# ValentinoGuerrini/Configurable-Hierarchical-Allreduce-Algorithms

Measured on AMD Instinct MI355X. Metric: device-resident bucket-reduction GB/s (fp32); allreduce GB/s at 2/4/8 GPUs, higher is better.
Workload: dtype f32; 1 GPU; C2 bucket reduction: k=2 (m=1 incoming bucket), 64 MiB fp32 per bucket, device-resident, MPI_Reduce_local semantics; bucket_bytes=67108864, m=1, buffer_sets=16, parallelism=replicas, gate=untimed spin kernel ahead of the start event

## Files before the change

### configurable-hierarchical-allreduce-algorithms_amd/csrc/reduce_kernels.hip

```cpp
#include <hip/hip_runtime.h>

#include <algorithm>

#include <cstdlib>

#include "reduce_vec.hpp"

namespace chr {

int& coresident_depth() {
    static thread_local int depth = 0;
    return depth;
}

ReduceTuning& reduce_tuning() {
    static ReduceTuning t = [] {
        ReduceTuning r;
        const char* s = std::getenv("CHR_REDUCE_MAX_LAUNCH_VEC");
        r.max_launch_vec = s ? (size_t)std::atoll(s) : 0;
        s = std::getenv("CHR_XCD_RUN_KIB");
        r.xcd_run_kib = s ? std::atoi(s) : -1;
        s = std::getenv("CHR_REDUCE_NT");
        r.nt_mode = s ? std::atoi(s) : -1;
        s = std::getenv("CHR_REDUCE_NT_MIN_BYTES");
        r.nt_min_bytes = s ? (size_t)std::atoll(s) : (size_t)40 << 20;
        r.tree_nt_min_bytes = s ? r.nt_min_bytes : (size_t)64 << 20;
        s = std::getenv("CHR_WG_PER_CU_VEC");
        r.wg_per_cu_vec = s ? std::max(0, std::atoi(s)) : -1;
        s = std::getenv("CHR_WG_PER_CU_TREE");
        r.wg_per_cu_tree = s ? std::max(0, std::atoi(s)) : -1;
        s = std::getenv("CHR_XCD_HAND_SHIFT");
        r.xcd_hand_shift = s ? std::min(31, std::max(0, std::atoi(s))) : -1;
        int dev = 0, lds = 0, blk = 0;
        if (hipGetDevice(&dev) != hipSuccess ||
            hipDeviceGetAttribute(&lds, hipDeviceAttributeMaxSharedMemoryPerMultiprocessor, dev) != hipSuccess ||
            lds <= 0)
            lds = 0;
        if (hipDeviceGetAttribute(&blk, hipDeviceAttributeMaxSharedMemoryPerBlock, dev) != hipSuccess || blk <= 0)
            blk = 0;
        r.lds_per_cu = (unsigned)lds;
        r.lds_per_block = (unsigned)blk;
        return r;
    }();
    return t;
}


static hipError_t launch_vec(const VecArgs& a, int kdt, int kop, int m, hipStream_t s) {
    kdt = vec_kernel_dt(kdt, kop);
    switch (kernel_tu(false, kdt, kop)) {
    case kTuCore: return launch_vec_tu<kTuCore>(a, kdt, kop, m, s);
    case kTuInt: return launch_vec_int(a, kdt, kop, m, s);
    case kTuPair: return launch_vec_pair(a, kdt, kop, m, s);
    default: return hipErrorInvalidValue;
    }
}

static hipError_t launch_scalar(void* out, const void* acc, const void* const* ins, int m, size_t n, int kdt,
                                int kop, hipStream_t s) {
    if (n == 0) return hipSuccess;
    ScalarArgs a{};
    a.out = out;
    a.acc = acc;
    a.m = m;
    a.n = n;
    for (int j = 0; j < m; ++j) a.ins[j] = ins[j];
    switch (kernel_tu(false, kdt, kop)) {
    case kTuCore: return launch_scalar_tu<kTuCore>(a, kdt, kop, s);
    case kTuInt: return launch_scalar_int(a, kdt, kop, s);
    case kTuPair: return launch_scalar_pair(a, kdt, kop, s);
    default: return hipErrorInvalidValue;
    }
}

static hipError_t launch_group(void* out, const void* acc, const void* const* ins, int m, size_t n, int dtype,
                               int op, hipStream_t s) {
    const size_t es = dtype_size(dtype);
    const void* operands[kMaxFanIn + 1] = {acc};
    for (int j = 0; j < m; ++j) operands[j + 1] = ins[j];
    const AlignSplit sp = align_split(out, operands, m + 1, n, es);
    if (!sp.congruent) return launch_scalar(out, acc, ins, m, n, dtype, op, s);
    hipError_t err;
    if (sp.head && (err = launch_scalar(out, acc, ins, m, sp.head, dtype, op, s)) != hipSuccess) return err;
    if (sp.nvec) {
        VecArgs a{};
        a.out = (u32x4*)((char*)out + sp.head * es);
        a.acc = (const u32x4*)((const char*)acc + sp.head * es);
        for (int j = 0; j < m; ++j) a.ins[j] = (const u32x4*)((const char*)ins[j] + sp.head * es);
        a.nvec = sp.nvec;
        if ((err = launch_vec(a, dtype, op, m, s)) != hipSuccess) return err;
    }
    if (sp.tail) {
        const size_t o = (n - sp.tail) * es;
        const void* tins[kMaxFanIn];
        for (int j = 0; j < m; ++j) tins[j] = (const char*)ins[j] + o;
        return launch_scalar((char*)out + o, (const char*)acc + o, tins, m, sp.tail, dtype, op, s);
    }
    return hipSuccess;
}

hipError_t launch_reduce(void* out, const void* acc, const void* const* ins, int m, size_t n, int dtype, int op,
                         hipStream_t stream, bool running_first) {
    if (n == 0) return hipSuccess;
    if (!valid_dtype_op(dtype, op)) return hipErrorInvalidValue;
    const size_t es = dtype_size(dtype);
    const KernelId k = canon_op(dtype, op, running_first);
    dtype = k.dt, op = k.op;
    if (m == 0) {
        if (out == acc) return hipSuccess;
        return hipMemcpyAsync(out, acc, n * es, hipMemcpyDeviceToDevice, stream);
    }
    for (int j0 = 0; j0 < m; j0 += kMaxFanIn) {
        const int mg = (m - j0) < kMaxFanIn ? (m - j0) : kMaxFanIn;
        hipError_t err = launch_group(out, j0 == 0 ? acc : out, ins + j0, mg, n, dtype, op, stream);
        if (err != hipSuccess) return err;
    }
    return hipSuccess;
}


__device__ __forceinline__ uint64_t splitmix64(uint64_t x) {
    x += 0x9E3779B97F4A7C15ull;
    x = (x ^ (x >> 30)) * 0xBF58476D1CE4E5B9ull;
    x = (x ^ (x >> 27)) * 0x94D049BB133111EBull;
    return x ^ (x >> 31);
}

__device__ __forceinline__ float gen_f32(uint64_t seed, uint64_t rank, uint64_t i) {
    return (float)(splitmix64(seed ^ (rank << 40) ^ i) >> 40) * (1.0f / 8388608.0f) - 1.0f;
}
__device__ __forceinline__ double gen_f64(uint64_t seed, uint64_t rank, uint64_t i) {
    return (double)(splitmix64(seed ^ (rank << 40) ^ i) >> 11) * (1.0 / 4503599627370496.0) - 1.0;
}

__device__ void fill_pair(char* elem, int dtype, int pattern, uint64_t seed, uint64_t rank, uint64_t count_for_seq,
                          uint64_t g) {
    const float ft[8] = {0.0f, -0.0f, 1.0f, -1.0f, 0.0f, -0.0f, 0.5f, 0.0f};
    const uint64_t key = splitmix64(seed ^ (rank << 40) ^ g);
    const unsigned sel = (unsigned)(key >> 61);
    const uint32_t pay = (uint32_t)(rank + 1) & 0x3Fu;
    const int32_t small = (int32_t)(key >> 61) - 4;
    const int32_t idx = pattern == 1 ? (int32_t)rank : (int32_t)((key >> 32) & 0x3F);
    const int32_t seq = (int32_t)(uint32_t)(rank * count_for_seq + g);
    uint32_t w[4] = {0, 0, 0, 0};
    switch (dtype) {
    case CHR_FLOAT_INT: {
        const float v = pattern == 1 ? (float)seq : pattern == 2 ? ft[sel] : (float)small;
        w[0] = pattern == 2 && sel == 7 ? (0x7FC00000u | (pay << 16) | pay) : __float_as_uint(v);
        w[1] = (uint32_t)idx;
        break;
    }
    case CHR_DOUBLE_INT: {
        const double v = pattern == 1 ? (double)seq : pattern == 2 ? (double)ft[sel] : (double)small;
        const uint64_t u = pattern == 2 && sel == 7 ? (0x7FF8000000000000ull | ((uint64_t)pay << 40) | pay)
                                                     : (uint64_t)__double_as_longlong(v);
        w[0] = (uint32_t)u;
        w[1] = (uint32_t)(u >> 32);
        w[2] = (uint32_t)idx;
        break;
    }
    case CHR_LONG_INT: {
        const uint64_t u = (uint64_t)(int64_t)(pattern == 1 ? seq : small);
        w[0] = (uint32_t)u;
        w[1] = (uint32_t)(u >> 32);
        w[2] = (uint32_t)idx;
        break;
    }
    case CHR_2INT:
        w[0] = (uint32_t)(pattern == 1 ? seq : small);
        w[1] = (uint32_t)idx;
        break;
    case CHR_SHORT_INT:
        w[0] = (uint32_t)(uint16_t)(int16_t)(pattern == 1 ? seq : small);
        w[1] = (uint32_t)idx;
        break;
    case CHR_C_FLOAT_COMPLEX: {
        const float re = pattern == 1 ? (float)seq : pattern == 2 ? ft[sel] : gen_f32(seed, rank, 2 * g);
        const float im = pattern == 1 ? -(float)seq : pattern == 2 ? ft[(key >> 58) & 7] : gen_f32(seed, rank, 2 * g + 1);
        w[0] = __float_as_uint(re);
        w[1] = __float_as_uint(im);
        break;
    }
    default: {
        const double re = pattern == 1 ? (double)seq : pattern == 2 ? (double)ft[sel] : gen_f64(seed, rank, 2 * g);
        const double im = pattern == 1 ? -(double)seq : pattern == 2 ? (double)ft[(key >> 58) & 7]
                                                                     : gen_f64(seed, rank, 2 * g + 1);
        const uint64_t ur = (uint64_t)__double_as_longlong(re), ui = (uint64_t)__double_as_longlong(im);
        w[0] = (uint32_t)ur;
        w[1] = (uint32_t)(ur >> 32);
        w[2] = (uint32_t)ui;
        w[3] = (uint32_t)(ui >> 32);
        break;
    }
    }
    const int nw = dtype == CHR_DOUBLE_INT || dtype == CHR_LONG_INT || dtype == CHR_C_DOUBLE_COMPLEX ? 4 : 2;
    for (int k = 0; k < nw; ++k) ((uint32_t*)elem)[k] = w[k];
}

__global__ __launch_bounds__(kBlock) void k_fill(void* buf, size_t n, int dtype, int pattern, uint64_t seed,
                                                 uint64_t rank, uint64_t count_for_seq) {
    if (dtype >= CHR_FLOAT_INT) {
        const size_t es = dtype == CHR_DOUBLE_INT || dtype == CHR_LONG_INT || dtype == CHR_C_DOUBLE_COMPLEX ? 16 : 8;
        for (size_t i = (size_t)blockIdx.x * kBlock + threadIdx.x; i < n; i += (size_t)gridDim.x * kBlock)
            fill_pair((char*)buf + i * es, dtype, pattern, seed, rank, count_for_seq, i);
        return;
    }
    const int es = dtype == CHR_INT8 || dtype == CHR_UINT8 ? 1 : dtype == CHR_INT16 || dtype == CHR_UINT16 ? 2
                   : dtype == CHR_UINT32 || (dtype == CHR_INT32 && pattern == 3) ? 4
                   : dtype == CHR_INT64 || dtype == CHR_UINT64 ? 8 : 0;
    for (size_t i = (size_t)blockIdx.x * kBlock + threadIdx.x; i < n; i += (size_t)gridDim.x * kBlock) {
        if (es) {
            const uint64_t u = splitmix64(seed ^ (rank << 40) ^ (uint64_t)i);
            const unsigned sel = (unsigned)(u >> 61);
            const uint64_t v = pattern == 1   ? rank * count_for_seq + i
                               : pattern == 2 ? (uint64_t)(int64_t)(sel == 6 ? 2 : sel == 7 ? 7 : sel == 2 ? 1
                                                                    : sel == 3 ? -1 : 0)
                               : pattern == 3 ? (sel ? (u >> (64 - 8 * es)) | 1u : 0)
                                              : u >> (64 - 8 * es);
            if (es == 1) ((uint8_t*)buf)[i] = (uint8_t)v;
            else if (es == 2) ((uint16_t*)buf)[i] = (uint16_t)v;
            else if (es == 4) ((uint32_t*)buf)[i] = (uint32_t)v;
            else ((uint64_t*)buf)[i] = v;
            continue;
        }
        if (pattern == 1) {
            const int32_t v = (int32_t)(uint32_t)(rank * count_for_seq + i);
            switch (dtype) {
            case CHR_FLOAT32: ((float*)buf)[i] = (float)v; break;
            case CHR_FLOAT64: ((double*)buf)[i] = (double)v; break;
            case CHR_INT32: ((int32_t*)buf)[i] = v; break;
            default: ((uint16_t*)buf)[i] = f2bf((float)v); break;
            }
        } else if (pattern == 2) {
            const unsigned sel = (unsigned)(splitmix64(seed ^ (rank << 40) ^ (uint64_t)i) >> 61);
            const uint32_t pay = (uint32_t)(rank + 1) & 0x3Fu;
            const float fv = sel == 2 ? 1.0f : sel == 3 ? -1.0f : sel == 6 ? 0.5f : (sel & 1) ? -0.0f : 0.0f;
            switch (dtype) {
            case CHR_FLOAT32:
                ((uint32_t*)buf)[i] = sel == 7 ? (0x7FC00000u | (pay << 16) | pay) : __float_as_uint(fv);
                break;
            case CHR_FLOAT64:
                ((uint64_t*)buf)[i] = sel == 7 ? (0x7FF8000000000000ull | ((uint64_t)pay << 40) | pay)
                                               : (uint64_t)__double_as_longlong((double)fv);
                break;
            case CHR_INT32: ((int32_t*)buf)[i] = sel == 6 ? 2 : sel == 7 ? 7 : sel == 2 ? 1 : sel == 3 ? -1 : 0; break;
            default: ((uint16_t*)buf)[i] = sel == 7 ? (uint16_t)(0x7FC0u | pay) : f2bf(fv); break;
            }
        } else {
            const uint64_t u = splitmix64(seed ^ (rank << 40) ^ (uint64_t)i);
            switch (dtype) {
            case CHR_FLOAT32: ((float*)buf)[i] = (float)(u >> 40) * (1.0f / 8388608.0f) - 1.0f; break;
            case CHR_FLOAT64: ((double*)buf)[i] = (double)(u >> 11) * (1.0 / 4503599627370496.0) - 1.0; break;
            case CHR_INT32: ((int32_t*)buf)[i] = (int32_t)(uint32_t)(u >> 32); break;
            default: ((uint16_t*)buf)[i] = f2bf((float)(u >> 40) * (1.0f / 8388608.0f) - 1.0f); break;
            }
        }
    }
}

hipError_t launch_fill(void* buf, size_t n, int dtype, int pattern, uint64_t seed, int rank, uint64_t count_for_seq,
                       hipStream_t stream) {
    if (n == 0) return hipSuccess;
    const size_t trips = (n + kBlock - 1) / kBlock;
    const int grid = (int)(trips < 8192 ? trips : 8192);
    hipLaunchKernelGGL(k_fill, dim3(grid), dim3(kBlock), 0, stream, buf, n, dtype, pattern, seed, (uint64_t)rank,
                       count_for_seq);
    return hipGetLastError();
}

}
```

### configurable-hierarchical-allreduce-algorithms_amd/csrc/reduce_tree.hip

```cpp
#include <hip/hip_runtime.h>

#include "reduce_tree.hpp"

namespace chr {

static hipError_t launch_tree_any(const TreeArgs& a, const TreeScalarArgs* sa, int kdt, int kop, hipStream_t s) {
    if (!sa) kdt = vec_kernel_dt(kdt, kop);
    switch (kernel_tu(true, kdt, kop)) {
    case kTuTree: return launch_tree_tu<kTuTree>(a, sa, kdt, kop, s);
    case kTuTreeIntNarrow: return launch_tree_int_narrow(a, sa, kdt, kop, s);
    case kTuTreeIntWide: return launch_tree_int_wide(a, sa, kdt, kop, s);
    case kTuTreePair: return launch_tree_pair(a, sa, kdt, kop, s);
    default: return hipErrorInvalidValue;
    }
}

bool tree_program_ok(int nl, const uint8_t* comb, const uint8_t* swaps, uint32_t* comb_bits, uint32_t* swap_bits) {
    if (nl < 1 || nl > kMaxLeaves || !comb) return false;
    int d = 0, nc = 0;
    uint32_t cb = 0, sb = 0;
    for (int j = 0; j < nl; ++j) {
        if (++d > kTreeDepth) return false;
        if ((int)comb[j] > d - 1) return false;
        cb |= (uint32_t)comb[j] << (2 * j);
        for (int c = 0; c < comb[j]; ++c, ++nc) {
            if (swaps && swaps[nc]) sb |= 1u << nc;
            --d;
        }
    }
    if (d != 1 || nc != nl - 1) return false;
    *comb_bits = cb;
    *swap_bits = sb;
    return true;
}

hipError_t launch_reduce_tree_multi(const TreeJob* jobs, int njobs, int dtype, int op, hipStream_t stream) {
    if (!valid_dtype_op(dtype, op)) return hipErrorInvalidValue;
    const size_t es = dtype_size(dtype);
    const int dtype0 = dtype, op0 = op;
    const KernelId k = canon_op(dtype, op, false);
    dtype = k.dt, op = k.op;
    TreeArgs pend[kMaxLeaves + 1] = {};
    auto flush = [&](int nl) -> hipError_t {
        TreeArgs& a = pend[nl];
        if (!a.nseg) return hipSuccess;
        a.nl = nl;
        const hipError_t e = launch_tree_any(a, nullptr, dtype, op, stream);
        a.nseg = 0;
        return e;
    };
    for (int t = 0; t < njobs; ++t) {
        const TreeJob& jb = jobs[t];
        if (jb.n == 0) continue;
        uint32_t cb = 0, sb = 0;
        if (!tree_program_ok(jb.nl, jb.comb, jb.swaps, &cb, &sb)) return hipErrorInvalidValue;
        const int nl = jb.nl;
        if (nl == 1) {
            if (jb.out != jb.leaves[0]) {
                const hipError_t e = hipMemcpyAsync(jb.out, jb.leaves[0], jb.n * es, hipMemcpyDeviceToDevice, stream);
                if (e != hipSuccess) return e;
            }
            continue;
        }
        if (nl == 2 && 3 * jb.n * es >= reduce_tuning().nt_min_bytes) {
            const bool sw = (sb & 1u) != 0;
            const void* acc = jb.leaves[sw ? 1 : 0];
            const void* in = jb.leaves[sw ? 0 : 1];
            if (jb.out != in) {
                const hipError_t e = launch_reduce(jb.out, acc, &in, 1, jb.n, dtype0, op0, stream);
                if (e != hipSuccess) return e;
                continue;
            }
        }
        const AlignSplit sp = align_split(jb.out, jb.leaves, nl, jb.n, es);
        const size_t head = sp.head, nvec = sp.nvec;
        auto scalar = [&](size_t off, size_t cnt) -> hipError_t {
            if (!cnt) return hipSuccess;
            TreeScalarArgs sa{};
            sa.out = (char*)jb.out + off * es;
            for (int j = 0; j < nl; ++j) sa.leaves[j] = (const char*)jb.leaves[j] + off * es;
            sa.n = cnt;
            sa.nl = nl;
            sa.comb = cb;
            sa.swaps = sb;
            TreeArgs dummy{};
            return launch_tree_any(dummy, &sa, dtype, op, stream);
        };
        hipError_t err;
        if (!sp.congruent) {
            if ((err = scalar(0, jb.n)) != hipSuccess) return err;
            continue;
        }
        if ((err = scalar(0, head)) != hipSuccess || (err = scalar(jb.n - sp.tail, sp.tail)) != hipSuccess) return err;
        const size_t cap = reduce_tuning().max_launch_vec;
        const size_t seg_cap = cap && cap < kMaxSegVec ? cap : kMaxSegVec;
        for (size_t off = 0; off < nvec; off += seg_cap) {
            TreeArgs& a = pend[nl];
            TreeSeg& g = a.seg[a.nseg++];
            g.out = (u32x4*)((char*)jb.out + head * es) + off;
            for (int j = 0; j < nl; ++j) g.leaves[j] = (const u32x4*)((const char*)jb.leaves[j] + head * es) + off;
            g.nvec = nvec - off < seg_cap ? nvec - off : seg_cap;
            g.comb = cb;
            g.swaps = sb;
            if (a.nseg == kMaxTreeSegs && (err = flush(nl)) != hipSuccess) return err;
        }
    }
    for (int nl = 2; nl <= kMaxLeaves; ++nl) {
        const hipError_t e = flush(nl);
        if (e != hipSuccess) return e;
    }
    return hipSuccess;
}

hipError_t launch_reduce_tree(void* out, const void* const* leaves, int nl, const uint8_t* comb, const uint8_t* swaps,
                              size_t n, int dtype, int op, hipStream_t stream) {
    if (n == 0) return hipSuccess;
    if (nl < 1 || nl > kMaxLeaves) return hipErrorInvalidValue;
    TreeJob jb{out, {}, nl, comb, swaps, n};
    for (int j = 0; j < nl; ++j) jb.leaves[j] = leaves[j];
    return launch_reduce_tree_multi(&jb, 1, dtype, op, stream);
}

}
```

### configurable-hierarchical-allreduce-algorithms_amd/csrc/reduce_vec.hpp

```cpp
#pragma once

#include <hip/hip_runtime.h>

#include "reduce_common.hpp"

namespace chr {

constexpr int kMaxFanIn = 8;

struct VecArgs {
    u32x4* out;
    const u32x4* acc;
    const u32x4* ins[kMaxFanIn];
    size_t nvec;
    uint32_t xrun;
    uint32_t xfull;
    uint32_t hand;
};

template <int DT, int OP, int M, int U, bool NT, bool ACC0, int BL>
__global__ __launch_bounds__(BL) void k_reduce_vec(VecArgs a) {
    u32x4* const out = a.out;
    const u32x4* const accp = a.acc;
    const u32x4* ins[M];
#pragma unroll
    for (int j = 0; j < M; ++j) ins[j] = a.ins[j];
    const size_t nvec = a.nvec;
    const uint32_t xrun = a.xrun, xfull = a.xfull, hand = a.hand;
    pin_sgpr(out, accp, nvec, xrun, xfull);
    pin_sgpr_u32(hand, hand);
#pragma unroll
    for (int j = 0; j < M; ++j) pin_sgpr(ins[j]);
    const size_t trip = xcd_trip_w(blockIdx.x, xfull, xrun, hand);
    if (trip == kIdleTrip) return;
    const size_t base = trip * BL * U + threadIdx.x;
    if ((trip + 1) * BL * U <= nvec) {
        u32x4 acc[U], x[M][U];
        acc[0] = ld<NT && !ACC0>(&accp[base]);
#pragma unroll
        for (int u = 1; u < U; ++u) acc[u] = ld<NT>(&accp[base + (size_t)u * BL]);
#pragma unroll
        for (int j = 0; j < M; ++j)
#pragma unroll
            for (int u = 0; u < U; ++u) x[j][u] = ld<NT>(&ins[j][base + (size_t)u * BL]);
        __builtin_amdgcn_sched_barrier(0);
#pragma unroll
        for (int j = 0; j < M; ++j)
#pragma unroll
            for (int u = 0; u < U; ++u) acc[u] = apply_vec<DT, OP>(x[j][u], acc[u]);
#pragma unroll
        for (int u = 0; u < U; ++u) st<NT>(&out[base + (size_t)u * BL], acc[u]);
    } else {
        for (int u = 0; u < U; ++u) {
            const size_t i = base + (size_t)u * BL;
            if (i >= nvec) break;
            u32x4 acc = accp[i];
#pragma unroll
            for (int j = 0; j < M; ++j) acc = apply_vec<DT, OP>(ins[j][i], acc);
            out[i] = acc;
        }
    }
}

struct ScalarArgs {
    void* out;
    const void* acc;
    const void* ins[kMaxFanIn];
    int m;
    size_t n;
};

template <int DT, int OP>
__global__ __launch_bounds__(kBlock) void k_reduce_scalar(ScalarArgs a) {
    using T = typename DTy<DT>::T;
    T* out = (T*)a.out;
    const T* acc = (const T*)a.acc;
    for (size_t i = (size_t)blockIdx.x * kBlock + threadIdx.x; i < a.n; i += (size_t)gridDim.x * kBlock) {
        T v = acc[i];
        for (int j = 0; j < a.m; ++j) v = apply<DT, OP>(((const T*)a.ins[j])[i], v);
        out[i] = v;
    }
}

template <int M>
constexpr size_t vec_xcd_run_kib() {
    return M <= 3 ? 256 : 512;
}

template <int M>
constexpr int vec_wg_per_cu() {
    return M == 2 ? 16 : 12;
}

template <int M>
constexpr int vec_u_nt() {
    return M == 1 ? 4 : M <= 3 ? 2 : 1;
}
template <int M, bool NT>
constexpr int vec_u() {
    return NT ? vec_u_nt<M>() : M <= 2 ? 4 : 2;
}
template <int DT, int OP, int M, bool NT>
constexpr int vec_u_dt() {
    return is_complex_dt<DT>() && (OP == CHR_PROD || OP == kProdSw) ? 1 : vec_u<M, NT>();
}

template <int BL, int U, bool WEIGHTED = false, typename L>
inline hipError_t for_each_launch_piece(VecArgs a, L launch) {
    const size_t cap = reduce_tuning().max_launch_vec;
    const size_t max_vec = cap ? cap : ((size_t)1 << 31) / BL * BL * U;
    for (size_t off = 0; off < a.nvec; off += max_vec) {
        VecArgs p = a;
        p.out = a.out + off;
        p.acc = a.acc + off;
        for (int j = 0; j < kMaxFanIn; ++j) p.ins[j] = a.ins[j] ? a.ins[j] + off : nullptr;
        p.nvec = a.nvec - off < max_vec ? a.nvec - off : max_vec;
        const unsigned trips = (unsigned)((p.nvec + (size_t)BL * U - 1) / ((size_t)BL * U));
        p.xfull = xcd_full(trips, p.xrun);
        p.hand = WEIGHTED ? xcd_hand(p.xfull, reduce_tuning().xcd_hand_shift) : 0u;
        launch(p, trips + 8u * p.hand);
        const hipError_t e = hipGetLastError();
        if (e != hipSuccess) return e;
    }
    return hipSuccess;
}

template <int DT, int OP, int M, int BL, bool NT, bool ACC0>
inline hipError_t launch_vec_mb_one(VecArgs a, hipStream_t s) {
    constexpr int U = vec_u_dt<DT, OP, M, NT>();
    a.xrun = NT ? xcd_run_shift(vec_xcd_run_kib<M>(), (size_t)BL * U * 16) : 0;
    const unsigned lds = NT ? nt_lds_bytes(reduce_tuning().wg_per_cu_vec, vec_wg_per_cu<M>()) : 0;
    return for_each_launch_piece<BL, U, NT>(a, [&](const VecArgs& p, unsigned grid) {
        hipLaunchKernelGGL((k_reduce_vec<DT, OP, M, U, NT, ACC0, BL>), dim3(grid), dim3(BL), lds, s, p);
    });
}

template <int DT, int OP, int M>
inline hipError_t launch_vec_m(const VecArgs& a, hipStream_t s) {
    if constexpr (is_pair_dt<DT>() || is_complex_dt<DT>()) {
        return launch_vec_mb_one<DT, OP, M, 256, false, false>(a, s);
    } else {
        const ReduceTuning& t = reduce_tuning();
        const size_t call_bytes = (size_t)(M + 2) * a.nvec * 16;
        const bool nt = t.nt_mode == 1 || (t.nt_mode < 0 && call_bytes >= t.nt_min_bytes);
        if (nt) return launch_vec_mb_one<DT, OP, M, 64, true, true>(a, s);
        return launch_vec_mb_one<DT, OP, M, 256, false, false>(a, s);
    }
}

template <int DT, int OP>
inline hipError_t launch_vec_op(const VecArgs& a, int m, hipStream_t s) {
    switch (m) {
    case 1: return launch_vec_m<DT, OP, 1>(a, s);
    case 2: return launch_vec_m<DT, OP, 2>(a, s);
    case 3: return launch_vec_m<DT, OP, 3>(a, s);
    case 4: return launch_vec_m<DT, OP, 4>(a, s);
    case 5: return launch_vec_m<DT, OP, 5>(a, s);
    case 6: return launch_vec_m<DT, OP, 6>(a, s);
    case 7: return launch_vec_m<DT, OP, 7>(a, s);
    case 8: return launch_vec_m<DT, OP, 8>(a, s);
    default: return hipErrorInvalidValue;
    }
}

template <int DT, int OP>
inline hipError_t launch_scalar_op(const ScalarArgs& a, hipStream_t s) {
    const size_t trips = (a.n + kBlock - 1) / kBlock;
    const int grid = (int)(trips < 2048 ? trips : 2048);
    hipLaunchKernelGGL((k_reduce_scalar<DT, OP>), dim3(grid), dim3(kBlock), 0, s, a);
    return hipGetLastError();
}

template <int TU>
inline hipError_t launch_vec_tu(const VecArgs& a, int kdt, int kop, int m, hipStream_t s) {
    return dispatch_kernel<TU>(kdt, kop, [&](auto dt, auto op) {
        constexpr int DT = decltype(dt)::value, OP = decltype(op)::value;
        if constexpr (vec_kernel_dt(DT, OP) != DT) return hipErrorInvalidValue;
        else return launch_vec_op<DT, OP>(a, m, s);
    });
}
template <int TU>
inline hipError_t launch_scalar_tu(const ScalarArgs& a, int kdt, int kop, hipStream_t s) {
    return dispatch_kernel<TU>(kdt, kop, [&](auto dt, auto op) {
        return launch_scalar_op<decltype(dt)::value, decltype(op)::value>(a, s);
    });
}

hipError_t launch_vec_int(const VecArgs& a, int kdt, int kop, int m, hipStream_t s);
hipError_t launch_scalar_int(const ScalarArgs& a, int kdt, int kop, hipStream_t s);
hipError_t launch_vec_pair(const VecArgs& a, int kdt, int kop, int m, hipStream_t s);
hipError_t launch_scalar_pair(const ScalarArgs& a, int kdt, int kop, hipStream_t s);

}
```

Measured before the change: 6718 GB/s.

## Add dynamic atomic tail-trip scheduling to the m=1 non-temporal reduce kernel

For the m=1 non-temporal vector reduce, the trailing portion of trips is no longer statically assigned. Extra blocks draw trip indices from sharded per-stream atomic counters, so work at the end of the launch balances across CUs/XCDs. A host-side lease gives out counter sets per stream or capture, with a generation tag and a host-mapped fault flag that disables the scheme on a mismatch. In exchange it adds per-block atomics, extra surplus blocks that exit immediately, and host mutex/lookup work per launch. The weighted XCD hand is turned off when the tail path is active.

```diff
diff --git a/configurable-hierarchical-allreduce-algorithms_amd/csrc/reduce_kernels.hip b/configurable-hierarchical-allreduce-algorithms_amd/csrc/reduce_kernels.hip
--- a/configurable-hierarchical-allreduce-algorithms_amd/csrc/reduce_kernels.hip
+++ b/configurable-hierarchical-allreduce-algorithms_amd/csrc/reduce_kernels.hip
@@ -1,8 +1,10 @@
 #include <hip/hip_runtime.h>
 
 #include <algorithm>
-
+#include <atomic>
 #include <cstdlib>
+#include <mutex>
+#include <unordered_map>
 
 #include "reduce_vec.hpp"
 
@@ -43,6 +45,98 @@
         return r;
     }();
     return t;
+}
+
+namespace {
+constexpr int kTailMaxDev = 64;
+struct TailPool {
+    std::atomic<bool> ready{false};
+    unsigned long long* sets = nullptr;
+    uint32_t* fault = nullptr;
+    bool off = false;
+    std::unordered_map<hipStream_t, uint32_t> by_stream;
+    uint32_t captured = 0;
+};
+TailPool g_tail_pool[kTailMaxDev];
+std::mutex g_tail_mu;
+std::atomic<uint32_t> g_tail_seq{0};
+
+bool tail_pool_make(TailPool& p, hipStream_t s) {
+    hipStreamCaptureMode mode = hipStreamCaptureModeRelaxed;
+    if (hipThreadExchangeStreamCaptureMode(&mode) != hipSuccess) {
+        (void)hipGetLastError();
+        return false;
+    }
+    const size_t bytes =
+        (size_t)(kTailStreamSets + kTailCapturedSets) * kTailShards * kTailStride * sizeof(unsigned long long);
+    unsigned long long* sets = nullptr;
+    uint32_t* fault = nullptr;
+    bool ok = hipMalloc(&sets, bytes) == hipSuccess &&
+              hipHostMalloc(&fault, sizeof(uint32_t), hipHostMallocPortable | hipHostMallocMapped) == hipSuccess;
+    if (ok) {
+        *fault = 0;
+        ok = hipMemsetAsync(sets, 0, bytes, s) == hipSuccess && hipStreamSynchronize(s) == hipSuccess;
+    }
+    (void)hipThreadExchangeStreamCaptureMode(&mode);
+    if (!ok) {
+        (void)hipGetLastError();
+        if (sets) (void)hipFree(sets);
+        if (fault) (void)hipHostFree(fault);
+        (void)hipGetLastError();
+        return false;
+    }
+    p.sets = sets;
+    p.fault = fault;
+    p.ready.store(true, std::memory_order_release);
+    return true;
+}
+}
+
+int& tail_static_depth() {
+    static thread_local int depth = 0;
+    return depth;
+}
+
+hipError_t tail_lease(hipStream_t s, uint32_t trips, TailLease* out) {
+    *out = TailLease{};
+    static const uint32_t min_trips = [] {
+        const char* e = std::getenv("CHR_TAIL_MIN_TRIPS");
+        return e ? (uint32_t)std::max(0ll, std::atoll(e)) : kTailMinTrips;
+    }();
+    if (trips < min_trips || coresident_depth() > 0 || tail_static_depth() > 0) return hipSuccess;
+    int dev = 0;
+    hipStreamCaptureStatus st = hipStreamCaptureStatusNone;
+    if (hipGetDevice(&dev) != hipSuccess || dev < 0 || dev >= kTailMaxDev ||
+        hipStreamIsCapturing(s, &st) != hipSuccess) {
+        (void)hipGetLastError();
+        return hipSuccess;
+    }
+    const bool capturing = st != hipStreamCaptureStatusNone;
+    TailPool& p = g_tail_pool[dev];
+    std::lock_guard<std::mutex> lock(g_tail_mu);
+    if (!p.ready.load(std::memory_order_acquire) && (capturing || !tail_pool_make(p, s))) return hipSuccess;
+    if (*(volatile uint32_t*)p.fault) {
+        *(volatile uint32_t*)p.fault = 0;
+        p.off = true;
+        return hipErrorLaunchFailure;
+    }
+    if (p.off) return hipSuccess;
+    uint32_t set;
+    if (capturing) {
+        if (p.captured >= kTailCapturedSets) return hipSuccess;
+        set = kTailStreamSets + p.captured++;
+    } else {
+        auto it = p.by_stream.find(s);
+        if (it == p.by_stream.end()) {
+            if (p.by_stream.size() >= kTailStreamSets) return hipSuccess;
+            it = p.by_stream.emplace(s, (uint32_t)p.by_stream.size()).first;
+        }
+        set = it->second;
+    }
+    out->ctr = p.sets + (size_t)set * kTailShards * kTailStride;
+    out->fault = p.fault;
+    out->gen = tail_gen(g_tail_seq.fetch_add(1, std::memory_order_relaxed));
+    return hipSuccess;
 }
 
 
diff --git a/configurable-hierarchical-allreduce-algorithms_amd/csrc/reduce_tree.hip b/configurable-hierarchical-allreduce-algorithms_amd/csrc/reduce_tree.hip
--- a/configurable-hierarchical-allreduce-algorithms_amd/csrc/reduce_tree.hip
+++ b/configurable-hierarchical-allreduce-algorithms_amd/csrc/reduce_tree.hip
@@ -3,6 +3,8 @@
 #include "reduce_tree.hpp"
 
 namespace chr {
+
+int& tail_static_depth();
 
 static hipError_t launch_tree_any(const TreeArgs& a, const TreeScalarArgs* sa, int kdt, int kop, hipStream_t s) {
     if (!sa) kdt = vec_kernel_dt(kdt, kop);
@@ -67,7 +69,9 @@
             const void* acc = jb.leaves[sw ? 1 : 0];
             const void* in = jb.leaves[sw ? 0 : 1];
             if (jb.out != in) {
+                ++tail_static_depth();
                 const hipError_t e = launch_reduce(jb.out, acc, &in, 1, jb.n, dtype0, op0, stream);
+                --tail_static_depth();
                 if (e != hipSuccess) return e;
                 continue;
             }
diff --git a/configurable-hierarchical-allreduce-algorithms_amd/csrc/reduce_vec.hpp b/configurable-hierarchical-allreduce-algorithms_amd/csrc/reduce_vec.hpp
--- a/configurable-hierarchical-allreduce-algorithms_amd/csrc/reduce_vec.hpp
+++ b/configurable-hierarchical-allreduce-algorithms_amd/csrc/reduce_vec.hpp
@@ -16,23 +16,110 @@
     uint32_t xrun;
     uint32_t xfull;
     uint32_t hand;
-};
+    uint32_t tail, extra;
+    uint32_t gen;
+    unsigned long long* ctr;
+    uint32_t* fault;
+};
+
+constexpr uint32_t kTailShards = 8, kTailStride = 16, kTailStreamSets = 256, kTailCapturedSets = 4096;
+constexpr int kTailShift = 4, kTailExtraShift = 5;
+constexpr uint32_t kTailMaxTrips = 1024, kTailMaxExtra = 512;
+constexpr uint32_t kTailMinTrips = 0;
+
+__host__ __device__ __forceinline__ uint32_t tail_count(uint32_t len, uint32_t k, uint32_t S = kTailShards) {
+    const uint32_t r = len % (8u * S), lo = 8u * k;
+    return len / (8u * S) * 8u + (r <= lo ? 0u : r - lo < 8u ? r - lo : 8u);
+}
+__host__ __device__ __forceinline__ uint32_t tail_shard(uint32_t j, uint32_t S = kTailShards) {
+    return (j >> 3) & (S - 1u);
+}
+__host__ __device__ __forceinline__ uint32_t tail_trip(uint32_t k, uint32_t idx, uint32_t S = kTailShards) {
+    return ((idx >> 3) * S + k) * 8u + (idx & 7u);
+}
+struct TailSplit {
+    uint32_t xfull, tail, extra;
+};
+inline TailSplit tail_split(uint32_t trips, uint32_t cs) {
+    constexpr int shift = kTailShift, extra_shift = kTailExtraShift;
+    const uint32_t want = trips >> shift < kTailMaxTrips ? trips >> shift : kTailMaxTrips;
+    const uint32_t b0 = xcd_full(trips - want, cs), n = trips - b0;
+    const uint32_t e = trips >> extra_shift < kTailMaxExtra ? trips >> extra_shift : kTailMaxExtra;
+    return {b0, n, n ? e : 0u};
+}
+__host__ __device__ __forceinline__ uint32_t tail_gen(uint32_t seq) { return (seq << 1 | 1u) * 2654435761u; }
+
+struct TailDraw {
+    uint32_t trip;
+    bool take;
+    bool reset;
+    bool fault;
+};
+__host__ __device__ __forceinline__ TailDraw tail_decide(unsigned long long draw, uint32_t j, uint32_t tail,
+                                                         uint32_t extra, uint32_t gen, uint32_t S = kTailShards) {
+    const uint32_t k = tail_shard(j, S), lo = (uint32_t)draw, hi = (uint32_t)(draw >> 32);
+    const uint32_t n = tail_count(tail, k, S), c = tail_count(tail + extra, k, S);
+    if (hi == lo * gen && lo < c) return {tail_trip(k, lo, S), lo < n, lo == c - 1u, false};
+    return {j, j < tail, false, true};
+}
+__device__ __forceinline__ unsigned long long tail_draw(unsigned long long* ctr, uint32_t j, uint32_t gen,
+                                                        uint32_t S = kTailShards) {
+    return __hip_atomic_fetch_add(&ctr[tail_shard(j, S) * kTailStride], 1ull | (unsigned long long)gen << 32,
+                                  __ATOMIC_RELAXED, __HIP_MEMORY_SCOPE_AGENT);
+}
+__device__ __forceinline__ void tail_reset(unsigned long long* ctr, uint32_t j, uint32_t S = kTailShards) {
+    __hip_atomic_store(&ctr[tail_shard(j, S) * kTailStride], 0ull, __ATOMIC_RELAXED, __HIP_MEMORY_SCOPE_AGENT);
+}
+
+struct TailLease {
+    unsigned long long* ctr;
+    uint32_t* fault;
+    uint32_t gen;
+};
+hipError_t tail_lease(hipStream_t s, uint32_t trips, TailLease* out);
+int& tail_static_depth();
+
+template <int M>
+constexpr bool vec_draws_tail() {
+    return M == 1;
+}
 
 template <int DT, int OP, int M, int U, bool NT, bool ACC0, int BL>
 __global__ __launch_bounds__(BL) void k_reduce_vec(VecArgs a) {
+    constexpr bool DRAW = NT && vec_draws_tail<M>();
     u32x4* const out = a.out;
     const u32x4* const accp = a.acc;
     const u32x4* ins[M];
 #pragma unroll
     for (int j = 0; j < M; ++j) ins[j] = a.ins[j];
     const size_t nvec = a.nvec;
-    const uint32_t xrun = a.xrun, xfull = a.xfull, hand = a.hand;
+    const uint32_t xrun = a.xrun, xfull = a.xfull;
+    const bool drawn = DRAW && a.tail != 0 && blockIdx.x >= xfull;
+    const uint32_t tj = blockIdx.x - xfull;
+    unsigned long long draw = 0;
+    if constexpr (DRAW) {
+        if (drawn && threadIdx.x == 0) draw = tail_draw(a.ctr, tj, a.gen);
+    }
     pin_sgpr(out, accp, nvec, xrun, xfull);
+    const uint32_t hand = a.hand;
     pin_sgpr_u32(hand, hand);
 #pragma unroll
     for (int j = 0; j < M; ++j) pin_sgpr(ins[j]);
-    const size_t trip = xcd_trip_w(blockIdx.x, xfull, xrun, hand);
+    size_t trip = xcd_trip_w(blockIdx.x, xfull, xrun, hand);
     if (trip == kIdleTrip) return;
+    if constexpr (DRAW) {
+        if (drawn) {
+            const uint32_t lo = (uint32_t)__builtin_amdgcn_readfirstlane((int)(uint32_t)draw);
+            const uint32_t hi = (uint32_t)__builtin_amdgcn_readfirstlane((int)(uint32_t)(draw >> 32));
+            const TailDraw d = tail_decide((unsigned long long)hi << 32 | lo, tj, a.tail, a.extra, a.gen);
+            if (threadIdx.x == 0) {
+                if (d.reset) tail_reset(a.ctr, tj);
+                if (d.fault) __hip_atomic_store(a.fault, 1u, __ATOMIC_RELAXED, __HIP_MEMORY_SCOPE_SYSTEM);
+            }
+            if (!d.take) return;
+            trip = (size_t)xfull + d.trip;
+        }
+    }
     const size_t base = trip * BL * U + threadIdx.x;
     if ((trip + 1) * BL * U <= nvec) {
         u32x4 acc[U], x[M][U];
@@ -105,8 +192,8 @@
     return is_complex_dt<DT>() && (OP == CHR_PROD || OP == kProdSw) ? 1 : vec_u<M, NT>();
 }
 
-template <int BL, int U, bool WEIGHTED = false, typename L>
-inline hipError_t for_each_launch_piece(VecArgs a, L launch) {
+template <int BL, int U, bool TAIL = false, bool WEIGHTED = false, typename L>
+inline hipError_t for_each_launch_piece(VecArgs a, hipStream_t s, L launch) {
     const size_t cap = reduce_tuning().max_launch_vec;
     const size_t max_vec = cap ? cap : ((size_t)1 << 31) / BL * BL * U;
     for (size_t off = 0; off < a.nvec; off += max_vec) {
@@ -117,8 +204,19 @@
         p.nvec = a.nvec - off < max_vec ? a.nvec - off : max_vec;
         const unsigned trips = (unsigned)((p.nvec + (size_t)BL * U - 1) / ((size_t)BL * U));
         p.xfull = xcd_full(trips, p.xrun);
+        p.tail = p.extra = 0;
         p.hand = WEIGHTED ? xcd_hand(p.xfull, reduce_tuning().xcd_hand_shift) : 0u;
-        launch(p, trips + 8u * p.hand);
+        if constexpr (TAIL) {
+            TailLease l{};
+            const hipError_t le = tail_lease(s, trips, &l);
+            if (le != hipSuccess) return le;
+            if (l.ctr) {
+                const TailSplit t = tail_split(trips, p.xrun);
+                p.xfull = t.xfull, p.tail = t.tail, p.extra = t.extra, p.hand = 0;
+                p.ctr = l.ctr, p.fault = l.fault, p.gen = l.gen;
+            }
+        }
+        launch(p, trips + p.extra + 8u * p.hand);
         const hipError_t e = hipGetLastError();
         if (e != hipSuccess) return e;
     }
@@ -130,7 +228,8 @@
     constexpr int U = vec_u_dt<DT, OP, M, NT>();
     a.xrun = NT ? xcd_run_shift(vec_xcd_run_kib<M>(), (size_t)BL * U * 16) : 0;
     const unsigned lds = NT ? nt_lds_bytes(reduce_tuning().wg_per_cu_vec, vec_wg_per_cu<M>()) : 0;
-    return for_each_launch_piece<BL, U, NT>(a, [&](const VecArgs& p, unsigned grid) {
+    constexpr bool DRAW = NT && vec_draws_tail<M>();
+    return for_each_launch_piece<BL, U, DRAW, NT>(a, s, [&](const VecArgs& p, unsigned grid) {
         hipLaunchKernelGGL((k_reduce_vec<DT, OP, M, U, NT, ACC0, BL>), dim3(grid), dim3(BL), lds, s, p);
     });
 }
```

After: 6798 GB/s (median of 6 runs). +1.2%, better.
